# aa2il/pySDR

Measured on AMD Instinct MI355X. Metric: complex IQ MS/s through 4-RX demod chain, higher is better.
Workload: dtype f32; 1 GPU; C3: 8 MS/s synthetic IQ, 4 RX (USB/CW/NFM/AM), 255-tap prototype 3/500, + 64k-FFT RF PSD on every sample; 2048 chunks x 170666 in HBM; parallelism=stream-sharded x1

## Files before the change

include/pysdr_hip.h:

```cpp
#ifndef PYSDR_HIP_H
#define PYSDR_HIP_H

#include <stddef.h>
#include <stdint.h>

#ifdef __cplusplus
extern "C" {
#endif

#define PYSDR_MAX_RX 8

typedef enum {
  PYSDR_OK = 0,
  PYSDR_ERR_ARG = -1,
  PYSDR_ERR_NO_DEVICE = -2,
  PYSDR_ERR_HIP = -3,
  PYSDR_ERR_FFT = -4,
  PYSDR_ERR_STATE = -5,
  PYSDR_ERR_RCCL = -6
} pysdr_status;

typedef enum {
  PYSDR_AM = 0, PYSDR_AM_SYNCH = 1, PYSDR_SSB = 2, PYSDR_USB = 3, PYSDR_LSB = 4,
  PYSDR_CW = 5, PYSDR_IQ = 6, PYSDR_WFM = 7, PYSDR_WFM2 = 8, PYSDR_NFM = 9,
// ... 42 lines not shown
int pysdr_wfm_params(double srate, double fs_out, int* d1, int* up2, int* down2);
int pysdr_set_wfm_taps(pysdr_ctx* ctx, int irx, const double* video, int nv, const double* resamp, int nr);
int pysdr_reset(pysdr_ctx* ctx, int irx, unsigned what);
int pysdr_agc_get(pysdr_ctx* ctx, int irx, pysdr_agc_state* st);
int pysdr_pll_stats(pysdr_ctx* ctx, int irx, int* segments, int* patched);
int pysdr_set_pll_segments(pysdr_ctx* ctx, int max_segments);
int pysdr_pll_join_margin(pysdr_ctx* ctx, int irx, int* max_words, float* max_dw);
int pysdr_pll_linear_starts(pysdr_ctx* ctx, int irx, int* n);
int pysdr_set_squelch(pysdr_ctx* ctx, int irx, float thresh);
int pysdr_squelch_get(pysdr_ctx* ctx, int irx, float* level, int* open);
int pysdr_set_squelch_ratio(pysdr_ctx* ctx, int irx, float min_ratio, const float* lp, const float* hp, int ntaps);
int pysdr_squelch_ratio_get(pysdr_ctx* ctx, int irx, float* sq_lp, float* sq_hp, int* open);
int pysdr_set_agc(pysdr_ctx* ctx, int irx, int enable, float ref);

int pysdr_process(pysdr_ctx* ctx, const float* iq_interleaved, size_t n, pysdr_out* outs);

int pysdr_process_batch(pysdr_ctx* ctx, const void* iq, int nchunks, size_t chunk_len, int on_device);
int pysdr_build_flags_hash(void);
int pysdr_set_overlap(pysdr_ctx* ctx, int enable);
int pysdr_get_overlap(pysdr_ctx* ctx);
int pysdr_last_call_overlapped(pysdr_ctx* ctx);
int pysdr_fetch(pysdr_ctx* ctx, int irx, float* am, float* iq, int cap, int* n_out,
                int* am_is_complex, int* chunk_nout, float* peaks);
int pysdr_sync(pysdr_ctx* ctx);

int pysdr_set_profile(pysdr_ctx* ctx, int enable);
int pysdr_get_elapsed_ms(pysdr_ctx* ctx, int which, int back, float* ms);
int pysdr_set_tile(pysdr_ctx* ctx, int tile_bytes, int threads);
int pysdr_get_tuning(pysdr_ctx* ctx, int32_t out[8]);

#define PYSDR_FORM_VECTOR 0
#define PYSDR_FORM_MFMA 1
#define PYSDR_FORM_SMALL 2
int pysdr_front_end_plan(int nrx, int up, int down, int ntaps, int tile_bytes, int threads, int wgs_per_cu,
                         int yflush_cap, int mfma_enable, int want_peak, int32_t out[12]);
int pysdr_front_end_shapes(int family, int index, int32_t out[4], int* count);

int pysdr_quad_mixer(int device, const float* x, float* y, size_t n, uint32_t phase0,
                     uint32_t fword, uint32_t* phase_out);
uint32_t pysdr_freq_word(double f_hz, double fs_hz, double* f_actual);

int pysdr_fir_real(int device, const float* xx, const float* h, int ntaps, float* y, size_t n);

int  pysdr_spectrum_create(int device, int chunk_size, int nfft, int max_frames,
                           const float* window, pysdr_spectrum** out);
void pysdr_spectrum_destroy(pysdr_spectrum* sp);
int pysdr_spectrum_frame(pysdr_spectrum* sp, const float* x, int is_complex, int db,
                         float* psd_out, int* n_out);
int pysdr_spectrum_batch(pysdr_spectrum* sp, const void* d_iq, int nframes, size_t hop,
                         void* d_out);
int pysdr_spectrum_sync(pysdr_spectrum* sp);
int pysdr_spectrum_get_tuning(pysdr_spectrum* sp, int32_t out[4]);
// ... 59 lines not shown
```

pysdr_amd/_lib.py:

```python
from __future__ import annotations

import ctypes as C
import os

HERE = os.path.dirname(os.path.abspath(__file__))
_variant = os.environ.get("PYSDR_LIB_VARIANT", "") if os.environ.get("PYSDR_TUNING", "0") not in ("", "0") else ""
LIB_PATH = os.path.join(HERE, "libpysdr_hip_diag.so" if os.environ.get("PYSDR_USE_DIAG_LIB") == "1"
                        else (f"libpysdr_hip_{_variant}.so" if _variant else "libpysdr_hip.so"))

MAX_RX = 8


class PysdrError(RuntimeError):
    pass


class Cfg(C.Structure):
    _fields_ = [("srate", C.c_double), ("up", C.c_int32), ("down", C.c_int32),
                ("in_chunk", C.c_int32), ("max_chunks", C.c_int32),
                ("ntaps_dec", C.c_int32), ("ntaps_af", C.c_int32),
                ("device", C.c_int32), ("reserved", C.c_int32)]


class AgcState(C.Structure):
# ... 26 lines not shown
    "pysdr_reset": (_i, [_vp, _i, C.c_uint]),
    "pysdr_agc_get": (_i, [_vp, _i, C.POINTER(AgcState)]),
    "pysdr_pll_stats": (_i, [_vp, _i, _pi, _pi]),
    "pysdr_set_pll_segments": (_i, [_vp, _i]),
    "pysdr_build_flags_hash": (_i, []),
    "pysdr_set_overlap": (_i, [_vp, _i]),
    "pysdr_get_overlap": (_i, [_vp]),
    "pysdr_last_call_overlapped": (_i, [_vp]),
    "pysdr_pll_join_margin": (_i, [_vp, _i, _pi, _pf]),
    "pysdr_pll_linear_starts": (_i, [_vp, _i, _pi]),
    "pysdr_set_agc": (_i, [_vp, _i, _i, _f]),
    "pysdr_set_squelch": (_i, [_vp, _i, _f]),
    "pysdr_squelch_get": (_i, [_vp, _i, _pf, _pi]),
    "pysdr_set_squelch_ratio": (_i, [_vp, _i, _f, _pf, _pf, _i]),
    "pysdr_squelch_ratio_get": (_i, [_vp, _i, _pf, _pf, _pi]),
    "pysdr_process": (_i, [_vp, _pf, _sz, C.POINTER(Out)]),
    "pysdr_process_batch": (_i, [_vp, _vp, _i, _sz, _i]),
    "pysdr_fetch": (_i, [_vp, _i, _pf, _pf, _i, _pi, _pi, _pi, _pf]),
    "pysdr_sync": (_i, [_vp]),
    "pysdr_set_profile": (_i, [_vp, _i]),
    "pysdr_get_elapsed_ms": (_i, [_vp, _i, _i, _pf]),
    "pysdr_set_tile": (_i, [_vp, _i, _i]),
    "pysdr_get_tuning": (_i, [_vp, C.POINTER(C.c_int32)]),
    "pysdr_front_end_plan": (_i, [_i, _i, _i, _i, _i, _i, _i, _i, _i, _i, C.POINTER(C.c_int32)]),
    "pysdr_front_end_shapes": (_i, [_i, _i, C.POINTER(C.c_int32), _pi]),
    "pysdr_quad_mixer": (_i, [_i, _pf, _pf, _sz, _u32, _u32, C.POINTER(_u32)]),
    "pysdr_freq_word": (_u32, [_d, _d, _pd]),
    "pysdr_fir_real": (_i, [_i, _pf, _pf, _i, _pf, _sz]),
    "pysdr_spectrum_create": (_i, [_i, _i, _i, _i, _pf, C.POINTER(_vp)]),
    "pysdr_spectrum_destroy": (None, [_vp]),
    "pysdr_spectrum_frame": (_i, [_vp, _pf, _i, _i, _pf, _pi]),
    "pysdr_spectrum_batch": (_i, [_vp, _vp, _i, _sz, _vp]),
    "pysdr_spectrum_sync": (_i, [_vp]),
    "pysdr_spectrum_get_tuning": (_i, [_vp, C.POINTER(C.c_int32)]),
    "pysdr_spectrum_elapsed_ms": (_i, [_vp, _pf]),
    "pysdr_spectrum_order": (_i, [_vp, _vp, _i]),
    "pysdr_ingest_create": (_i, [_vp, _i, C.POINTER(_vp)]),
    "pysdr_ingest_create_batched": (_i, [_vp, _i, _i, C.POINTER(_vp)]),
    "pysdr_ingest_chunks": (_i, [_vp, _i, _i, _pi, _pi, _pf]),
    "pysdr_ingest_destroy": (None, [_vp]),
    "pysdr_ingest_buffer": (_i, [_vp, _i, C.POINTER(_pf), C.POINTER(C.c_size_t)]),
    "pysdr_ingest_submit": (_i, [_vp, _i, C.c_size_t]),
    "pysdr_ingest_collect": (_i, [_vp, _i, C.POINTER(Out)]),
    "pysdr_waterfall_create": (_i, [_i, _i, _i, C.POINTER(_vp)]),
    "pysdr_waterfall_destroy": (None, [_vp]),
    "pysdr_waterfall_push": (_i, [_vp, _vp, _i, _i]),
# ... 79 lines not shown
```

pysdr_amd/csrc/api.hip:

```cpp
#include <dlfcn.h>
#include <rccl/rccl.h>
#include <rocfft/rocfft.h>

#include <cmath>
#include <algorithm>
#include <cstdarg>
#include <map>

#include "common.h"
#include "host_plan.h"
#include "host_res.h"
#include "mixdec_mfma_geom.h"
#include "mixdec_plan.h"

namespace pysdr {

static thread_local char g_err[2048] = "";

void set_last_error(const char* fmt, ...) {
  va_list ap;
  va_start(ap, fmt);
  vsnprintf(g_err, sizeof(g_err), fmt, ap);
  va_end(ap);
}
// ... 104 lines not shown
  bool use2 = false;
  int par = 0;
  int last_par = 0;
  Event ev_pll[2];
  int n_ingest = 0;
  TailJob tail;
  int hy = 0, mmax = 0;
  size_t cap_samples = 0;
  Decim main;
  Decim wfm_front;
  int d1 = 0, up2 = 0, down2 = 0, m1max = 0;
  int last_wfm = 0;
  DevBuf<float2> d_stage;
  BufPair<unsigned> d_peak2;
  int peak_cur = 0;
  bool peak_clean[2] = {true, true};
#ifdef PYSDR_DIAG
  DevBuf<unsigned long long> d_stamps;
  DevBuf<unsigned long long> d_mm_stamps;
#endif
  DevBuf<unsigned> d_peak_scratch;
  DevBuf<unsigned> d_blkpeak;
  DevBuf<float> d_gain;
  DevBuf<float> d_blknoise;
  DevBuf<float> d_blknoise2;
  DevBuf<float> d_sqtaps;
  int sq_ntaps = 0;
  DevBuf<unsigned> d_blkcnt;
  DevBuf<RxDevState> d_state;
  DevBuf<uint32_t> d_pllseg;
  int last_nout = 0, last_nchunks = 0, last_nrx = 0;
  size_t last_chunk_len = 0;
  unsigned long long last_s0 = 0;
  int last_complex[PYSDR_MAX_RX] = {0};
  Tuning tune;
  int num_cus = 256;
  int pll_kmax = 0;
  int profile = 0;
  static constexpr int kSlots = 64;
  Event ev[kSlots][4];
  Event ev_front;
  hipEvent_t front_marker = nullptr;
  int front_wanted = 0;
  unsigned long long ncalls = 0;
  void* rccl_lib = nullptr;
  ncclComm_t comm = nullptr;
// ... 356 lines not shown
  const double wn = 2.0 * M_PI * kPllBwHz / fs_out;
  s.pll_kp = (float)(2.0 * kPllZeta * wn);
  s.pll_ki = (float)(wn * wn);
  for (int r = 0; r < nrx; ++r) {
    const RxSnap& x = snap.rx[r];
    s.y[r] = x.d_y + c->hy;
    s.ypll[r] = x.d_ypll ? x.d_ypll + c->hy : nullptr;
    s.aftaps[r] = x.d_aftaps;
    s.taps_real[r] = x.taps_real;
    s.a[r] = x.d_a;
    s.am[r] = x.d_am;
    s.det[r] = mode_detector(x.mode);
    s.out_complex[r] = (x.mode == PYSDR_IQ || wfm) ? 1 : 0;
    s.fir_complex[r] = s.out_complex[r];
    s.single_block[r] = wfm ? 1 : 0;
    s.single_spread = 1;
    while (s.single_spread * 2 <= std::min(nchunks, 32)) s.single_spread *= 2;
    s.matrix[r] = (x.mode == PYSDR_WFM2) ? 1 : 0;
    s.bfo_fword[r] = x.bfo_fword;
    s.sq_ratio[r] = (x.sq_ratio > 0.f && c->d_sqtaps) ? 1 : 0;
    s.sq_thresh[r] = s.sq_ratio[r] ? x.sq_ratio : x.sq_thresh;
  }
  s.blkpeak = c->d_blkpeak.get(); s.gain = c->d_gain.get(); s.state = c->d_state.get();
  s.blknoise = c->d_blknoise.get(); s.blkcnt = c->d_blkcnt.get();
  s.blknoise2 = c->d_blknoise2.get(); s.sqtaps = c->d_sqtaps.get(); s.sq_ntaps = c->sq_ntaps;
}

int run_tail(pysdr_ctx* c, TailJob& j) {
  j.valid = false;
  const CallSnap& snap = j.snap;
  const int nrx = snap.nrx;
  if (j.wait_pll) PYSDR_HIP_CHECK(hipStreamWaitEvent(c->stream, c->ev_pll[j.par], 0));
  Stage2Args& s = j.s;
  int rc;
  if (j.wfm) {
    DecimResult res;
    const uint32_t zero = 0u;
    for (int r = 0; r < nrx; ++r) {
      float2* y1 = snap.rx[r].d_y + c->hy;
      rc = decim_run(c, c->rx[r].wfm_audio, snap.rx[r].d_w, (size_t)j.n1, 1, &y1, &zero, &zero, nullptr, 0,
                     c->mmax, &res, c->stream);
      if (rc) return rc;
    }
    fill_stage2(c, snap, true, j.nchunks, j.chunk_len, res, &s);
  }
  const int n_out = s.n_out;
// ... 20 lines not shown
}

int flush_tail(pysdr_ctx* c) {
  if (!c->tail.valid) return PYSDR_OK;
  return run_tail(c, c->tail);
}

int failed_in(const char* entry, int rc) {
  const std::string what = pysdr_last_error();
  set_last_error("%s: %s", entry, what.c_str());
  return rc;
}

int ctx_alloc(pysdr_ctx* c) {
  const pysdr_cfg& cfg = c->cfg;
  const size_t nblk = (size_t)PYSDR_MAX_RX * cfg.max_chunks;
  PYSDR_HIP_CHECK(c->stream.create(hipStreamNonBlocking));
  int rc = decim_init(c->main, cfg.up, cfg.down, cfg.ntaps_dec, PYSDR_MAX_RX, c->stream);
  if (rc) return rc;
  PYSDR_HIP_CHECK(c->d_peak2.alloc_both_zeroed((size_t)cfg.max_chunks, c->stream));
  PYSDR_HIP_CHECK(c->d_peak_scratch.alloc(64));
  PYSDR_HIP_CHECK(c->d_blkpeak.alloc_zeroed(nblk * kBlkStride, c->stream));
  PYSDR_HIP_CHECK(c->d_gain.alloc(nblk));
  PYSDR_HIP_CHECK(c->d_blknoise.alloc_zeroed(nblk * kBlkStride, c->stream));
  PYSDR_HIP_CHECK(c->d_blkcnt.alloc_zeroed(nblk * kBlkStride, c->stream));
  PYSDR_HIP_CHECK(c->d_state.alloc_zeroed(PYSDR_MAX_RX, c->stream));
  PYSDR_HIP_CHECK(c->d_pllseg.alloc((size_t)PYSDR_MAX_RX * kPllSegMax * 5));
  for (int k = 0; k < pysdr_ctx::kSlots; ++k)
    for (int i = 0; i < 4; ++i) PYSDR_HIP_CHECK(c->ev[k][i].create());
  PYSDR_HIP_CHECK(c->ev_front.create(hipEventDisableTiming));
  return PYSDR_OK;
}

int read_rx_state(pysdr_ctx* c, int irx, RxDevState* d) {
  if (!c || irx < 0 || irx >= c->nrx) return PYSDR_ERR_ARG;
  std::lock_guard<std::recursive_mutex> run_lk(c->run_mu);
  int rc = use_device(c->cfg.device);
  if (rc) return rc;
  rc = flush_tail(c);
  if (rc) return rc;
  PYSDR_HIP_CHECK(hipMemcpyAsync(d, c->d_state.get() + irx, sizeof(*d), hipMemcpyDeviceToHost, c->stream));
  PYSDR_HIP_CHECK(hipStreamSynchronize(c->stream));
  return PYSDR_OK;
}

}
// ... 276 lines not shown
#endif

int pysdr_build_flags_hash(void) {
#ifdef PYSDR_EXTRA_FLAGS_HASH
  return (int)(PYSDR_EXTRA_FLAGS_HASH);
#else
  return 0;
#endif
}

int pysdr_get_tuning(pysdr_ctx* c, int32_t out[8]) {
  if (!c || !out) return PYSDR_ERR_ARG;
#ifdef PYSDR_DIAG
  out[0] = 1;
#else
  out[0] = 0;
#endif
  const Tuning& t = c->tune;
  out[1] = t.dbg_flags; out[2] = t.wgs_per_cu; out[3] = t.yflush_cap;
  out[4] = t.tile_bytes; out[5] = t.threads; out[6] = c->num_cus; out[7] = t.mfma_enable;
  return PYSDR_OK;
}

int pysdr_set_profile(pysdr_ctx* c, int enable) {
  if (!c) return PYSDR_ERR_ARG;
  c->profile = enable;
  return PYSDR_OK;
}

int pysdr_set_tile(pysdr_ctx* c, int tile_bytes, int threads) {
  if (!c || (tile_bytes != 0 && (tile_bytes < 4096 || tile_bytes > 150 * 1024)) || threads < 64 || threads > 1024 ||
      (threads & 63))
    return PYSDR_ERR_ARG;
  c->tune.tile_bytes = tile_bytes;
  c->tune.threads = threads;
  return PYSDR_OK;
}

int pysdr_front_end_plan(int nrx, int up, int down, int ntaps, int tile_bytes, int threads, int wgs_per_cu, int yflush_cap,
                         int mfma_enable, int want_peak, int32_t out[12]) {
  if (!out || nrx < 1 || nrx > PYSDR_MAX_RX || up < 1 || down < 1 || ntaps < 1 || wgs_per_cu < 1 || yflush_cap < 0 ||
      (tile_bytes != 0 && (tile_bytes < 4096 || tile_bytes > 150 * 1024)) || threads < 64 || threads > 1024 || (threads & 63))
    return PYSDR_ERR_ARG;
  const int kdec = (ntaps + up - 1) / up;
  MixDecArgs a;
  memset(&a, 0, sizeof(a));
// ... 285 lines not shown
int pysdr_fetch(pysdr_ctx* c, int irx, float* am, float* iq, int cap, int* n_out,
                int* am_is_complex, int* chunk_nout, float* peaks) {
  if (!c || irx < 0 || irx >= c->nrx) return PYSDR_ERR_ARG;
  std::lock_guard<std::recursive_mutex> run_lk(c->run_mu);
  int rc = use_device(c->cfg.device);
  if (rc) return rc;
  rc = flush_tail(c);
  if (rc) return rc;
  const int n = c->last_nout;
  if ((am || iq) && cap < n) { set_last_error("pysdr_fetch: cap %d < n_out %d", cap, n); return PYSDR_ERR_ARG; }
  const int cx = c->last_complex[irx];
  hipStream_t S2 = c->stream;
  const float2* yb = c->rx[irx].d_y.buf(c->last_par);
  if (am && n > 0)
    PYSDR_HIP_CHECK(hipMemcpyAsync(am, c->rx[irx].d_am.get(), (size_t)n * (cx ? 2 : 1) * sizeof(float), hipMemcpyDeviceToHost, S2));
  if (iq && n > 0)
    PYSDR_HIP_CHECK(hipMemcpyAsync(iq, yb + c->hy, (size_t)n * sizeof(float2), hipMemcpyDeviceToHost, S2));
  if (peaks && c->last_nchunks > 0)
    PYSDR_HIP_CHECK(hipMemcpyAsync(peaks, c->d_peak2.buf(c->peak_cur), (size_t)c->last_nchunks * sizeof(float), hipMemcpyDeviceToHost, S2));
  PYSDR_HIP_CHECK(hipStreamSynchronize(S2));
  if (n_out) *n_out = n;
  if (am_is_complex) *am_is_complex = cx;
  if (chunk_nout) last_chunk_counts(c, chunk_nout);
  return PYSDR_OK;
}

int pysdr_process(pysdr_ctx* c, const float* iq, size_t n, pysdr_out* outs) {
  if (!c || !iq || !outs || n < 1) return PYSDR_ERR_ARG;
  std::lock_guard<std::recursive_mutex> run_lk(c->run_mu);
  int rc = pysdr_process_batch(c, iq, 1, n, 0);
  if (rc) return rc;
  rc = flush_tail(c);
  if (rc) return rc;
  for (int r = 0; r < c->last_nrx; ++r) {
    int nout = 0, cx = 0;
    float pk = 0.f;
    rc = pysdr_fetch(c, r, outs[r].am, outs[r].iq, outs[r].cap, &nout, &cx, nullptr, &pk);
    if (rc) return rc;
    outs[r].n_out = nout;
    outs[r].am_is_complex = cx;
    outs[r].peak_in = pk;
  }
  return PYSDR_OK;
}

int pysdr_quad_mixer(int device, const float* x, float* y, size_t n, uint32_t phase0,
// ... 524 lines not shown
```

pysdr_amd/csrc/common.h:

```cpp
#pragma once

#include <hip/hip_runtime.h>

#include <cstdint>
#include <cstdio>
#include <cstring>
#include <mutex>
#include <string>
#include <vector>

#include "../../include/pysdr_hip.h"

#if defined(PYSDR_GLDS_PLAIN)
#define PYSDR_GLDS_POLICY ""
#else
#define PYSDR_GLDS_POLICY " nt"
#endif

namespace pysdr {

void set_last_error(const char* fmt, ...);

#define PYSDR_HIP_CHECK(expr)                                                        \
  do {                                                                               \
// ... 102 lines not shown
#define PYSDR_MFMA_SHAPES(X) \
  X(0, 3, 128, 2, 334, 1, 8, MM_C1_NPROD, MM_C1_NBUF, MM_C1_FLAGS) \
  X(1, 1, 40, MM_C4_S, 255, 1, 8, MM_C4_NPROD, MM_C4_NBUF, MM_C4_FLAGS) \
  X(2, 3, 64, 2, 334, 1, 8, 8, 4, 1 | MM_NTX) \
  X(3, 3, 160, 2, 334, 1, 8, 8, 3, 2 | MM_NTX) \
  X(4, 3, 112, 2, 334, 1, 8, 8, 4, 1 | MM_NTX) \
  X(5, 1, 32, 8, 1001, 1, 8, 4, 3, 0 | MM_NTX) \
  X(6, 1, 40, 6, 1001, 1, 8, 4, 3, 0 | MM_NTX)
inline int mixdec_mfma_shape(int up, int down, int kdec) {
#define PYSDR_MFMA_MATCH(ID, UP, DOWN, S, KT, NB, WK, NP, NBUF, CARRY) \
  if (up == UP && down == DOWN && kdec == KT) return ID;
  PYSDR_MFMA_SHAPES(PYSDR_MFMA_MATCH)
#undef PYSDR_MFMA_MATCH
  return -1;
}
bool mixdec_mfma_plan(int shape, unsigned long long s0, unsigned long long m0, unsigned long long n, MfmaPlan* p);
int launch_mixdec_mfma(int shape, const MixMfmaArgs& a, int grid, hipStream_t st);


#ifndef PYSDR_BLK_STRIDE
#define PYSDR_BLK_STRIDE 16
#endif
constexpr int kBlkStride = PYSDR_BLK_STRIDE;

struct RxDevState {
  float env, gain, maxbuf, err, ref;
  int agc_enable;
  uint32_t pll_phase;
  float pll_w;
  uint32_t wfm_phase;
  float wfm_w;
  float sq_level;
  int sq_open;
  int pll_segments;
  int pll_patched;
  int pll_join_words;
  float pll_join_dw;
  int pll_linear;
  int wfm_slope_ok;
  int wfm_redo;
  double wfm_slope;
  float sq_lp, sq_hp;
};
constexpr int kSqTapsMax = 64;
constexpr float kSqAlpha = 0.001f;
constexpr float kSqLog2Decay = -0.00144341686f;
// ... 23 lines not shown
  float2* ypll[PYSDR_MAX_RX];
  const float2* aftaps[PYSDR_MAX_RX];
  int taps_real[PYSDR_MAX_RX];
  float2* a[PYSDR_MAX_RX];
  float* am[PYSDR_MAX_RX];
  int det[PYSDR_MAX_RX];
  int out_complex[PYSDR_MAX_RX];
  int fir_complex[PYSDR_MAX_RX];
  int fir_rx[PYSDR_MAX_RX];
  uint32_t bfo_fword[PYSDR_MAX_RX];
  int single_block[PYSDR_MAX_RX];
  int single_spread;
  int matrix[PYSDR_MAX_RX];
  float sq_thresh[PYSDR_MAX_RX];
  int sq_ratio[PYSDR_MAX_RX];
  int sq_ntaps;
  const float* sqtaps;
  float* blknoise2;
  float* blknoise;
  unsigned* blkcnt;
  unsigned* blkpeak;
  float* gain;
  RxDevState* state;
  PllPlan pll;
};
int launch_am_phase(const Stage2Args& a, hipStream_t st);
int launch_pll(const Stage2Args& a, hipStream_t st);
int launch_demod_fir(const Stage2Args& a, hipStream_t st);
int launch_apply(const Stage2Args& a, hipStream_t st);

struct EpilogueArgs {
  int nrx, n_out, hy;
  float2* ybase[PYSDR_MAX_RX];
  float2* ydst[PYSDR_MAX_RX];
  float2* ypllbase[PYSDR_MAX_RX];
  float2* yplldst[PYSDR_MAX_RX];
};
int launch_agc_scan(const Stage2Args& a, const EpilogueArgs& e, hipStream_t st);
int launch_hist_roll(const float2* x, const float2* hist_old, float2* hist_new, int hist_len,
                     uint32_t n_total, unsigned* zero, int zero_n, hipStream_t st);

struct WfmArgs {
  int nrx, n1;
  float scale;
  float kp, ki, norm, rad2word;
  uint32_t fword0;
  const float2* y1[PYSDR_MAX_RX];
  float2* y1base[PYSDR_MAX_RX];
// ... 33 lines not shown
```

pysdr_amd/csrc/host_plan.h:

```cpp
#pragma once

#include <algorithm>
#include <cmath>
#include <cstdlib>

#include "common.h"

namespace pysdr {

constexpr double kTwo32 = 4294967296.0;
constexpr double kPllBwHz = 50.0, kPllZeta = 0.7071;
constexpr double kWfmPllBwHz = 30.0;
constexpr int kPllSegMax = 8192;

inline const char* tuning_env(const char* name) {
  const char* on = getenv("PYSDR_TUNING");
  if (!on || atoi(on) <= 0) return nullptr;
  return getenv(name);
}

struct Tuning {
  int tile_bytes = 0, threads = 1024;
  int wgs_per_cu = 1;
  int grid_override = 0;
  int resamp_plain = 0;
  int mfma_enable = 1;
  int dbg_flags = 0, yflush_cap = 0;
  int overlap_env = -1;
  int tail_first = -1;
  bool overlap_prio_set = false;
  int overlap_prio = 0;
  double am_taus = 16.0, am_taus_exact = 5.0;
  int am_coarse_sweeps = 4, am_kmax = 2048, am_tmin = 512;
  int am_seeded = 1, am_wseed = 0;
  int am_direct = 1;
  int am_phase_on_2 = 1;
  double wfm_taus = 20.0, wfm_taus_fast = 13.0, wfm_taus_exact = 4.0;
  int wfm_coarse_sweeps = 3, wfm_kmax = 1536, wfm_tmin = 2048;
  double wfm_taus_hi = 0.0, wfm_taus_mid = 0.0;
  int wfm_tail_cap = 0;
  int wfm_exact_cap = 5;
  int wfm_seeded = 1, wfm_wseed = 0;

  static Tuning from_env() {
    Tuning t;
    { const char* e = tuning_env("PYSDR_MIXDEC_WGS"); if (e && atoi(e) > 0) t.wgs_per_cu = atoi(e); }
    { const char* e = tuning_env("PYSDR_MIXDEC_YFLUSH"); if (e && atoi(e) > 0) t.yflush_cap = atoi(e); }
    { const char* e = tuning_env("PYSDR_AM_PLL");
      if (e && *e) {
        double a = 0, tx = 0; int cs = 0, km = 0, tm = 0;
        const int nf = sscanf(e, "%lf,%lf,%d,%d,%d", &a, &tx, &cs, &km, &tm);
        if (nf >= 1 && a > 0) t.am_taus = a;
        if (nf >= 2 && tx >= 0) t.am_taus_exact = tx;
        if (nf >= 3 && cs >= 0) t.am_coarse_sweeps = std::min(cs, 8);
        if (nf >= 4 && km > 0) t.am_kmax = std::min(km, kPllSegMax);
        if (nf >= 5 && tm >= 64) t.am_tmin = (tm + 63) & ~63;
      } }
    { const char* e = tuning_env("PYSDR_AM_SEED");
      if (e && *e) { int on = 1, ws = 0; const int nf = sscanf(e, "%d,%d", &on, &ws); if (nf >= 1) t.am_seeded = on ? 1 : 0; if (nf >= 2 && ws >= 0) t.am_wseed = ws; } }
    { const char* e = tuning_env("PYSDR_AM_DIRECT"); if (e && *e) t.am_direct = atoi(e) ? 1 : 0; }
    { const char* e = tuning_env("PYSDR_AM_PHASE_STREAM"); if (e && *e) t.am_phase_on_2 = atoi(e) ? 1 : 0; }
    { const char* e = tuning_env("PYSDR_MIXDEC_MFMA"); if (e && *e) t.mfma_enable = atoi(e) ? 1 : 0; }
    { const char* e = tuning_env("PYSDR_WFM_SEED");
      if (e && *e) { int on = 1, ws = 0; const int nf = sscanf(e, "%d,%d", &on, &ws); if (nf >= 1) t.wfm_seeded = on ? 1 : 0; if (nf >= 2 && ws >= 0) t.wfm_wseed = ws; } }
    { const char* e = tuning_env("PYSDR_OVERLAP_ORDER"); if (e && *e) t.tail_first = atoi(e); }
    { const char* e = tuning_env("PYSDR_OVERLAP"); if (e && *e) t.overlap_env = std::max(0, std::min(2, atoi(e))); }
    { const char* e = tuning_env("PYSDR_OVERLAP_PRIO"); if (e && *e) { t.overlap_prio_set = true; t.overlap_prio = atoi(e); } }
    { const char* e = tuning_env("PYSDR_RESAMP_PLAIN"); if (e && *e) t.resamp_plain = atoi(e); }
    { const char* e = tuning_env("PYSDR_MIXDEC_GRID"); if (e && atoi(e) > 0) t.grid_override = atoi(e); }
    { const char* e = tuning_env("PYSDR_WFM_PLL");
      if (e && *e) {
        double a = t.wfm_taus, b = t.wfm_taus_fast, x = t.wfm_taus_exact;
        int sw = t.wfm_coarse_sweeps, km = t.wfm_kmax, tm = t.wfm_tmin, xc = t.wfm_exact_cap;
        double th = t.wfm_taus_hi, tmid = t.wfm_taus_mid;
        int tc = t.wfm_tail_cap;
        const int got = sscanf(e, "%lf,%lf,%lf,%d,%d,%d,%d,%lf,%lf,%d", &a, &b, &x, &sw, &km, &tm, &xc, &th, &tmid, &tc);
        if (got >= 10 && tc >= 0) t.wfm_tail_cap = tc;
        if (got >= 9 && th >= 0 && tmid >= 0) { t.wfm_taus_hi = th; t.wfm_taus_mid = tmid; }
        if (got >= 7 && xc >= 0) t.wfm_exact_cap = xc;
        if (got >= 1 && a > 0) t.wfm_taus = a;
        if (got >= 2 && b >= 0) t.wfm_taus_fast = b;
        if (got >= 3 && x > 0) t.wfm_taus_exact = x;
        if (got >= 4 && sw >= 0) t.wfm_coarse_sweeps = sw;
        if (got >= 5 && km >= 1) t.wfm_kmax = std::min(km, kPllSegMax);
        if (got >= 6 && tm >= 64) t.wfm_tmin = tm;
      } }
#ifdef PYSDR_DIAG
    { const char* e = getenv("PYSDR_DEBUG_FLAGS"); t.dbg_flags = e ? atoi(e) : 0; }
#endif
    return t;
  }
// ... 95 lines not shown
```

pysdr_amd/csrc/stage2.hip:

```cpp
#include "common.h"
#include "hist_roll.h"

namespace pysdr {

namespace {

__device__ __forceinline__ float2 cmul(float2 a, float2 b) {
  return make_float2(a.x * b.x - a.y * b.y, a.x * b.y + a.y * b.x);
}

__device__ __forceinline__ uint32_t block_of(const Stage2Args& a, int r, int i) {
  if (a.single_block[r]) return 0u;
  const uint32_t t = a.t0 + (uint32_t)i * (uint32_t)a.down;
  return (t / (uint32_t)a.up) / a.chunk_len;
}

__device__ __forceinline__ int block_end(const Stage2Args& a, int r, uint32_t b) {
  if (a.single_block[r] || b + 1u >= (uint32_t)a.nchunks) return a.n_out;
  const unsigned long long need = (unsigned long long)(b + 1u) * a.chunk_len * (unsigned)a.up;
  if (need <= a.t0) return 0;
  const unsigned long long i = (need - a.t0 + (unsigned)a.down - 1ull) / (unsigned)a.down;
  return i < (unsigned long long)a.n_out ? (int)i : a.n_out;
}

// ... 670 lines not shown
  __syncthreads();

  float2 acc[kW];
  if (CPLX) {
    fir_run<kFirCplx>(sre, sim, tre, tim, tre_s, tim_s, nblk, H, tid, acc);
  } else {
    const bool real_det = (det == kDetAbs || det == kDetFm || det == kDetPll);
    if (real_det && a.taps_real[r]) fir_run<kFirRealReal>(sre, sim, tre, tim, tre_s, tim_s, nblk, H, tid, acc);
    else fir_run<kFirRePart>(sre, sim, tre, tim, tre_s, tim_s, nblk, H, tid, acc);
  }

  fir_epilogue<CPLX>(a, r, det, i0, H, tid, sre, acc);
}


__device__ __forceinline__ float agc_env_step(float env, float peak) {
  const float dec = __fadd_rn(env, __fmul_rn(0.1f, __fsub_rn(peak, env)));
  return (peak > env) ? peak : dec;
}

__global__ __launch_bounds__(256) void agc_scan_kernel(const Stage2Args a, const EpilogueArgs eh) {
  extern __shared__ __attribute__((aligned(16))) float agc_lds[];
  const int tid = threadIdx.x;
  if ((int)blockIdx.x >= a.nrx) {
    const int job = blockIdx.x - a.nrx;
    const float2* base = (job < eh.nrx) ? eh.ybase[job] : eh.ypllbase[job - eh.nrx];
    float2* dst = (job < eh.nrx) ? eh.ydst[job] : eh.yplldst[job - eh.nrx];
    if (base == nullptr) return;
    float2* sh = reinterpret_cast<float2*>(agc_lds);
    for (int j = tid; j < eh.hy; j += 256) sh[j] = base[eh.n_out + j];
    __syncthreads();
    for (int j = tid; j < eh.hy; j += 256) dst[j] = sh[j];
    return;
  }
  const int r = blockIdx.x;
  const int nch = a.single_block[r] ? (a.nchunks > 0 ? 1 : 0) : a.nchunks;
  const int nacc = a.single_block[r] ? (a.nchunks > 0 ? a.single_spread : 0) : a.nchunks;
  auto px = [](int c) { return c + (c >> 4); };
  const int nlds = px(a.nchunks) + 1;
  float* pk = agc_lds;
  float* ev = agc_lds + nlds;
  float* sS = ev + nlds;
  float* sE = sS + 256;
  for (int c0 = 0; c0 < nacc; c0 += 16 * 256) {
    unsigned v[16];
#pragma unroll
    for (int u = 0; u < 16; ++u) {
      const int c = c0 + u * 256 + tid;
      v[u] = (c < nacc) ? a.blkpeak[((size_t)r * a.nchunks + c) * kBlkStride] : 0u;
    }
#pragma unroll
    for (int u = 0; u < 16; ++u) {
      const int c = c0 + u * 256 + tid;
      if (c < nacc) pk[px(c)] = __uint_as_float(v[u]);
    }
  }
  __syncthreads();
  if (a.single_block[r] && nacc > 1) {
    if (tid == 0) {
      float m = pk[px(0)];
      for (int c = 1; c < nacc; ++c) m = fmaxf(m, pk[px(c)]);
      pk[px(0)] = m;
    }
    __syncthreads();
  }
  const RxDevState st = a.state[r];
  constexpr int kWarm = 176;
  const int T = (nch + 255) / 256 < 16 ? 16 : (nch + 255) / 256;
  const int K = (nch + T - 1) / T;
  if (tid < K) {
    const int s0 = tid * T, s1 = (s0 + T < nch) ? s0 + T : nch;
    int wb = s0 - kWarm;
    float env = 0.f;
    if (tid == 0 || wb <= 0) { wb = 0; env = st.env; }
    int c = wb;
    for (; c + 16 <= s0; c += 16) {
      float v[16];
#pragma unroll
      for (int u = 0; u < 16; ++u) v[u] = pk[px(c + u)];
#pragma unroll
      for (int u = 0; u < 16; ++u) env = agc_env_step(env, v[u]);
    }
    for (; c < s0; ++c) env = agc_env_step(env, pk[px(c)]);
    sS[tid] = env;
    for (c = s0; c + 16 <= s1; c += 16) {
      float v[16];
#pragma unroll
      for (int u = 0; u < 16; ++u) v[u] = pk[px(c + u)];
#pragma unroll
      for (int u = 0; u < 16; ++u) { env = agc_env_step(env, v[u]); ev[px(c + u)] = env; }
    }
    for (; c < s1; ++c) { env = agc_env_step(env, pk[px(c)]); ev[px(c)] = env; }
    sE[tid] = env;
  }
  __syncthreads();
  const bool miss = tid > 0 && tid < K && __float_as_uint(sE[tid - 1]) != __float_as_uint(sS[tid]);
  if (__syncthreads_or(miss) && tid == 0) {
    for (int k = 1; k < K; ++k) {
      if (__float_as_uint(sE[k - 1]) == __float_as_uint(sS[k])) continue;
      float env = sE[k - 1];
      const int s0 = k * T, s1 = (s0 + T < nch) ? s0 + T : nch;
      for (int c = s0; c < s1; ++c) { env = agc_env_step(env, pk[px(c)]); ev[px(c)] = env; }
      sE[k] = env;
      sS[k] = sE[k - 1];
    }
  }
  __syncthreads();
  const float last_peak = nch > 0 ? pk[px(nch - 1)] : st.maxbuf;
  for (int c = tid; c < nch; c += 256) pk[px(c)] = ev[px(c)];
  __syncthreads();
  for (int c = tid; c < nch; c += 256) {
    const float g = st.agc_enable ? fminf(__fdiv_rn(st.ref, fmaxf(pk[px(c)], 1e-12f)), 1.0e4f) : 1.f;
    a.gain[(size_t)r * a.nchunks + c] = g;
    a.blkpeak[((size_t)r * a.nchunks + c) * kBlkStride] = 0u;
  }
  if (a.single_block[r])
    for (int c = 1 + tid; c < nacc; c += 256) a.blkpeak[((size_t)r * a.nchunks + c) * kBlkStride] = 0u;
  const float env_last = nch > 0 ? pk[px(nch - 1)] : 0.f;
  if (a.sq_thresh[r] > 0.f && a.sq_ratio[r]) {
    constexpr int kSqWarm = 32;
    __syncthreads();
    float* wH = ev;
    float* wL = pk;
    float* dk = sE + 256;
    float* lvH = dk + nlds;
    float* lvL = lvH + nlds;
    float* sS2 = lvL + nlds;
    float* sE2 = sS2 + 256;
    for (int c = tid; c < nch; c += 256) {
      const size_t k = ((size_t)r * a.nchunks + c) * kBlkStride;
      const unsigned n = a.blkcnt[k];
// ... 487 lines not shown
                                          hipFuncAttributeMaxDynamicSharedMemorySize, 160 * 1024));
      attr_done |= 1ull << (dev & 63);
    }
  }
  for (int cplx = 0; cplx < 2; ++cplx) {
    Stage2Args b = a;
    int n = 0;
    for (int r = 0; r < a.nrx; ++r)
      if ((a.out_complex[r] ? 1 : 0) == cplx) b.fir_rx[n++] = r;
    if (n == 0) continue;
    dim3 grid((a.n_out + (int)(a.m0_lo & 1u) + kFirOut - 1) / kFirOut, n);
    if (cplx) hipLaunchKernelGGL(demod_fir_kernel<true>, grid, dim3(kFirThreads), lds, st, b);
    else hipLaunchKernelGGL(demod_fir_kernel<false>, grid, dim3(kFirThreads), lds, st, b);
    PYSDR_HIP_CHECK(hipGetLastError());
  }
  return PYSDR_OK;
}

int launch_agc_scan(const Stage2Args& a, const EpilogueArgs& e, hipStream_t st) {
  if (e.hy > 4096) {
    set_last_error("epilogue: history %d too long", e.hy);
    return PYSDR_ERR_ARG;
  }
  const size_t nlds = (size_t)a.nchunks + (a.nchunks >> 4) + 1;
  bool any_ratio = false;
  for (int r = 0; r < a.nrx; ++r) any_ratio |= (a.sq_ratio[r] != 0 && a.sq_thresh[r] > 0.f);
  const size_t lds = std::max(((any_ratio ? 5 : 2) * nlds + (any_ratio ? 1024 : 512)) * sizeof(float), (size_t)e.hy * sizeof(float2));
  if (lds > 48 * 1024) {
    static std::mutex attr_mu;
    static uint64_t attr_done = 0;
    static size_t max_dyn = 0;
    int dev = 0;
    PYSDR_HIP_CHECK(hipGetDevice(&dev));
    std::lock_guard<std::mutex> lk(attr_mu);
    if (max_dyn == 0) {
      hipFuncAttributes fa;
      PYSDR_HIP_CHECK(hipFuncGetAttributes(&fa, reinterpret_cast<const void*>(agc_scan_kernel)));
      max_dyn = (size_t)160 * 1024 - fa.sharedSizeBytes;
    }
    if (lds > max_dyn) { set_last_error("agc: %d blocks per call need %zu bytes of LDS (%zu available)", a.nchunks, lds, max_dyn); return PYSDR_ERR_ARG; }
    if (!((attr_done >> (dev & 63)) & 1ull)) {
      PYSDR_HIP_CHECK(hipFuncSetAttribute(reinterpret_cast<const void*>(agc_scan_kernel),
                                          hipFuncAttributeMaxDynamicSharedMemorySize, (int)max_dyn));
      attr_done |= 1ull << (dev & 63);
    }
  }
  hipLaunchKernelGGL(agc_scan_kernel, dim3(a.nrx + 2 * e.nrx), dim3(256), lds, st, a, e);
  PYSDR_HIP_CHECK(hipGetLastError());
  return PYSDR_OK;
}

int launch_apply(const Stage2Args& a, hipStream_t st) {
  if (a.n_out <= 0) return PYSDR_OK;
  dim3 grid((a.n_out + 1023) / 1024, a.nrx);
  hipLaunchKernelGGL(apply_kernel, grid, dim3(256), 0, st, a);
  PYSDR_HIP_CHECK(hipGetLastError());
  return PYSDR_OK;
}

int launch_hist_roll(const float2* x, const float2* hist_old, float2* hist_new, int hist_len,
                     uint32_t n_total, unsigned* zero, int zero_n, hipStream_t st) {
  hipLaunchKernelGGL(hist_roll_kernel, dim3(1), dim3(256), 0, st, x, hist_old, hist_new, hist_len, n_total, zero, zero_n);
  PYSDR_HIP_CHECK(hipGetLastError());
  return PYSDR_OK;
}

int launch_wfm_disc(const WfmArgs& a, hipStream_t st) {
  if (a.n1 > 0) {
    hipLaunchKernelGGL(wfm_disc_kernel, dim3((a.n1 + kSeedTile - 1) / kSeedTile, a.nrx), dim3(256), 0, st, a);
    PYSDR_HIP_CHECK(hipGetLastError());
// ... 41 lines not shown
```

Baseline: 118,300 MS/s.

## Split AGC envelope scan across several workgroups per receiver with last-block join

```diff
diff --git a/include/pysdr_hip.h b/include/pysdr_hip.h
--- a/include/pysdr_hip.h
+++ b/include/pysdr_hip.h
@@ -88,12 +88,14 @@
 int pysdr_last_call_overlapped(pysdr_ctx* ctx);
 int pysdr_fetch(pysdr_ctx* ctx, int irx, float* am, float* iq, int cap, int* n_out,
                 int* am_is_complex, int* chunk_nout, float* peaks);
+int pysdr_fetch_gains(pysdr_ctx* ctx, int irx, float* gains, int cap, int* nblocks);
 int pysdr_sync(pysdr_ctx* ctx);
 
 int pysdr_set_profile(pysdr_ctx* ctx, int enable);
 int pysdr_get_elapsed_ms(pysdr_ctx* ctx, int which, int back, float* ms);
 int pysdr_set_tile(pysdr_ctx* ctx, int tile_bytes, int threads);
 int pysdr_get_tuning(pysdr_ctx* ctx, int32_t out[8]);
+int pysdr_get_agc_scan(pysdr_ctx* ctx, int32_t out[4]);
 
 #define PYSDR_FORM_VECTOR 0
 #define PYSDR_FORM_MFMA 1
diff --git a/pysdr_amd/_lib.py b/pysdr_amd/_lib.py
--- a/pysdr_amd/_lib.py
+++ b/pysdr_amd/_lib.py
@@ -72,6 +72,8 @@
     "pysdr_get_elapsed_ms": (_i, [_vp, _i, _i, _pf]),
     "pysdr_set_tile": (_i, [_vp, _i, _i]),
     "pysdr_get_tuning": (_i, [_vp, C.POINTER(C.c_int32)]),
+    "pysdr_get_agc_scan": (_i, [_vp, C.POINTER(C.c_int32)]),
+    "pysdr_fetch_gains": (_i, [_vp, _i, _pf, _i, _pi]),
     "pysdr_front_end_plan": (_i, [_i, _i, _i, _i, _i, _i, _i, _i, _i, _i, C.POINTER(C.c_int32)]),
     "pysdr_front_end_shapes": (_i, [_i, _i, C.POINTER(C.c_int32), _pi]),
     "pysdr_quad_mixer": (_i, [_i, _pf, _pf, _sz, _u32, _u32, C.POINTER(_u32)]),
diff --git a/pysdr_amd/csrc/api.hip b/pysdr_amd/csrc/api.hip
--- a/pysdr_amd/csrc/api.hip
+++ b/pysdr_amd/csrc/api.hip
@@ -150,6 +150,9 @@
   DevBuf<unsigned> d_peak_scratch;
   DevBuf<unsigned> d_blkpeak;
   DevBuf<float> d_gain;
+  DevBuf<float> d_agcenv;
+  DevBuf<float> d_agcseg;
+  DevBuf<unsigned> d_agcjoin;
   DevBuf<float> d_blknoise;
   DevBuf<float> d_blknoise2;
   DevBuf<float> d_sqtaps;
@@ -552,6 +555,9 @@
     s.sq_thresh[r] = s.sq_ratio[r] ? x.sq_ratio : x.sq_thresh;
   }
   s.blkpeak = c->d_blkpeak.get(); s.gain = c->d_gain.get(); s.state = c->d_state.get();
+  s.agc_ranges = agc_scan_ranges(nchunks, c->tune.agc_ranges);
+  s.agc_env = c->d_agcenv.get(); s.agc_seg = c->d_agcseg.get();
+  s.agc_join = c->d_agcjoin.get(); s.agc_diag = c->d_agcjoin.get() + PYSDR_MAX_RX * kAgcJoinPitch;
   s.blknoise = c->d_blknoise.get(); s.blkcnt = c->d_blkcnt.get();
   s.blknoise2 = c->d_blknoise2.get(); s.sqtaps = c->d_sqtaps.get(); s.sq_ntaps = c->sq_ntaps;
 }
@@ -618,6 +624,9 @@
   PYSDR_HIP_CHECK(c->d_peak_scratch.alloc(64));
   PYSDR_HIP_CHECK(c->d_blkpeak.alloc_zeroed(nblk * kBlkStride, c->stream));
   PYSDR_HIP_CHECK(c->d_gain.alloc(nblk));
+  PYSDR_HIP_CHECK(c->d_agcenv.alloc(nblk));
+  PYSDR_HIP_CHECK(c->d_agcseg.alloc((size_t)PYSDR_MAX_RX * 2 * kAgcSegMax));
+  PYSDR_HIP_CHECK(c->d_agcjoin.alloc_zeroed((size_t)PYSDR_MAX_RX * kAgcJoinPitch + kAgcDiagWords, c->stream));
   PYSDR_HIP_CHECK(c->d_blknoise.alloc_zeroed(nblk * kBlkStride, c->stream));
   PYSDR_HIP_CHECK(c->d_blkcnt.alloc_zeroed(nblk * kBlkStride, c->stream));
   PYSDR_HIP_CHECK(c->d_state.alloc_zeroed(PYSDR_MAX_RX, c->stream));
@@ -940,6 +949,20 @@
   return PYSDR_OK;
 }
 
+int pysdr_get_agc_scan(pysdr_ctx* c, int32_t out[4]) {
+  if (!c || !out) return PYSDR_ERR_ARG;
+  std::lock_guard<std::recursive_mutex> run_lk(c->run_mu);
+  int rc = use_device(c->cfg.device);
+  if (rc) return rc;
+  rc = flush_tail(c);
+  if (rc) return rc;
+  unsigned diag[kAgcDiagWords];
+  PYSDR_HIP_CHECK(hipMemcpyAsync(diag, c->d_agcjoin.get() + PYSDR_MAX_RX * kAgcJoinPitch, sizeof(diag), hipMemcpyDeviceToHost, c->stream));
+  PYSDR_HIP_CHECK(hipStreamSynchronize(c->stream));
+  out[0] = c->tune.agc_ranges; out[1] = (int32_t)diag[0]; out[2] = (int32_t)diag[1]; out[3] = 0;
+  return PYSDR_OK;
+}
+
 int pysdr_set_profile(pysdr_ctx* c, int enable) {
   if (!c) return PYSDR_ERR_ARG;
   c->profile = enable;
@@ -1271,6 +1294,22 @@
   if (n_out) *n_out = n;
   if (am_is_complex) *am_is_complex = cx;
   if (chunk_nout) last_chunk_counts(c, chunk_nout);
+  return PYSDR_OK;
+}
+
+int pysdr_fetch_gains(pysdr_ctx* c, int irx, float* gains, int cap, int* nblocks) {
+  if (!c || irx < 0 || irx >= c->nrx) return PYSDR_ERR_ARG;
+  std::lock_guard<std::recursive_mutex> run_lk(c->run_mu);
+  int rc = use_device(c->cfg.device);
+  if (rc) return rc;
+  rc = flush_tail(c);
+  if (rc) return rc;
+  const int n = c->last_wfm ? (c->last_nchunks > 0 ? 1 : 0) : c->last_nchunks;
+  if (gains && cap < n) { set_last_error("pysdr_fetch_gains: cap %d < %d blocks", cap, n); return PYSDR_ERR_ARG; }
+  if (gains && n > 0)
+    PYSDR_HIP_CHECK(hipMemcpyAsync(gains, c->d_gain.get() + (size_t)irx * c->last_nchunks, (size_t)n * sizeof(float), hipMemcpyDeviceToHost, c->stream));
+  PYSDR_HIP_CHECK(hipStreamSynchronize(c->stream));
+  if (nblocks) *nblocks = n;
   return PYSDR_OK;
 }
 
diff --git a/pysdr_amd/csrc/common.h b/pysdr_amd/csrc/common.h
--- a/pysdr_amd/csrc/common.h
+++ b/pysdr_amd/csrc/common.h
@@ -148,6 +148,7 @@
 #define PYSDR_BLK_STRIDE 16
 #endif
 constexpr int kBlkStride = PYSDR_BLK_STRIDE;
+static_assert(kBlkStride >= 2 && kBlkStride % 2 == 0, "PYSDR_BLK_STRIDE: an even number of words, at least 2");
 
 struct RxDevState {
   float env, gain, maxbuf, err, ref;
@@ -217,8 +218,21 @@
   unsigned* blkpeak;
   float* gain;
   RxDevState* state;
+  int agc_ranges;
+  float* agc_env;
+  float* agc_seg;
+  unsigned* agc_join;
+  unsigned* agc_diag;
   PllPlan pll;
 };
+constexpr int kAgcSegMax = 256;
+constexpr int kAgcJoinPitch = 32;
+constexpr int kAgcDiagWords = 4;
+constexpr int kAgcRangesMax = 8;
+inline int agc_scan_ranges(int nchunks, int forced) {
+  const int j = forced > 0 ? forced : nchunks / 256;
+  return j < 1 ? 1 : (j > kAgcRangesMax ? kAgcRangesMax : j);
+}
 int launch_am_phase(const Stage2Args& a, hipStream_t st);
 int launch_pll(const Stage2Args& a, hipStream_t st);
 int launch_demod_fir(const Stage2Args& a, hipStream_t st);
diff --git a/pysdr_amd/csrc/host_plan.h b/pysdr_amd/csrc/host_plan.h
--- a/pysdr_amd/csrc/host_plan.h
+++ b/pysdr_amd/csrc/host_plan.h
@@ -24,6 +24,7 @@
   int wgs_per_cu = 1;
   int grid_override = 0;
   int resamp_plain = 0;
+  int agc_ranges = 0;
   int mfma_enable = 1;
   int dbg_flags = 0, yflush_cap = 0;
   int overlap_env = -1;
@@ -67,6 +68,7 @@
     { const char* e = tuning_env("PYSDR_OVERLAP"); if (e && *e) t.overlap_env = std::max(0, std::min(2, atoi(e))); }
     { const char* e = tuning_env("PYSDR_OVERLAP_PRIO"); if (e && *e) { t.overlap_prio_set = true; t.overlap_prio = atoi(e); } }
     { const char* e = tuning_env("PYSDR_RESAMP_PLAIN"); if (e && *e) t.resamp_plain = atoi(e); }
+    { const char* e = tuning_env("PYSDR_AGC_RANGES"); if (e && atoi(e) > 0) t.agc_ranges = atoi(e); }
     { const char* e = tuning_env("PYSDR_MIXDEC_GRID"); if (e && atoi(e) > 0) t.grid_override = atoi(e); }
     { const char* e = tuning_env("PYSDR_WFM_PLL");
       if (e && *e) {
diff --git a/pysdr_amd/csrc/stage2.hip b/pysdr_amd/csrc/stage2.hip
--- a/pysdr_amd/csrc/stage2.hip
+++ b/pysdr_amd/csrc/stage2.hip
@@ -716,8 +716,9 @@
 __global__ __launch_bounds__(256) void agc_scan_kernel(const Stage2Args a, const EpilogueArgs eh) {
   extern __shared__ __attribute__((aligned(16))) float agc_lds[];
   const int tid = threadIdx.x;
-  if ((int)blockIdx.x >= a.nrx) {
-    const int job = blockIdx.x - a.nrx;
+  const int J = a.agc_ranges;
+  if ((int)blockIdx.x >= a.nrx * J) {
+    const int job = blockIdx.x - a.nrx * J;
     const float2* base = (job < eh.nrx) ? eh.ybase[job] : eh.ypllbase[job - eh.nrx];
     float2* dst = (job < eh.nrx) ? eh.ydst[job] : eh.yplldst[job - eh.nrx];
     if (base == nullptr) return;
@@ -727,7 +728,7 @@
     for (int j = tid; j < eh.hy; j += 256) dst[j] = sh[j];
     return;
   }
-  const int r = blockIdx.x;
+  const int r = blockIdx.x / J, j = blockIdx.x - r * J;
   const int nch = a.single_block[r] ? (a.nchunks > 0 ? 1 : 0) : a.nchunks;
   const int nacc = a.single_block[r] ? (a.nchunks > 0 ? a.single_spread : 0) : a.nchunks;
   auto px = [](int c) { return c + (c >> 4); };
@@ -736,19 +737,32 @@
   float* ev = agc_lds + nlds;
   float* sS = ev + nlds;
   float* sE = sS + 256;
-  for (int c0 = 0; c0 < nacc; c0 += 16 * 256) {
-    unsigned v[16];
-#pragma unroll
-    for (int u = 0; u < 16; ++u) {
-      const int c = c0 + u * 256 + tid;
-      v[u] = (c < nacc) ? a.blkpeak[((size_t)r * a.nchunks + c) * kBlkStride] : 0u;
-    }
-#pragma unroll
-    for (int u = 0; u < 16; ++u) {
-      const int c = c0 + u * 256 + tid;
-      if (c < nacc) pk[px(c)] = __uint_as_float(v[u]);
-    }
-  }
+  auto load_peaks = [&](int lo, int hi) {
+    for (int c0 = lo; c0 < hi; c0 += 16 * 256) {
+      unsigned v[16];
+#pragma unroll
+      for (int u = 0; u < 16; ++u) {
+        const int c = c0 + u * 256 + tid;
+        v[u] = (c < hi) ? a.blkpeak[((size_t)r * a.nchunks + c) * kBlkStride] : 0u;
+      }
+#pragma unroll
+      for (int u = 0; u < 16; ++u) {
+        const int c = c0 + u * 256 + tid;
+        if (c < hi) pk[px(c)] = __uint_as_float(v[u]);
+      }
+    }
+  };
+  constexpr int kWarm = 176;
+  const int T = (nch + 255) / 256 < 16 ? 16 : (nch + 255) / 256;
+  const int K = (nch + T - 1) / T;
+  const int jr = (a.single_block[r] || K < 2) ? 1 : (J < K ? J : K);
+  const int spr = (K + jr - 1) / jr;
+  const int nranges = spr > 0 ? (K + spr - 1) / spr : 1;
+  if (j >= nranges) return;
+  const int k0 = j * spr, k1 = (k0 + spr < K) ? k0 + spr : K;
+  const int lo = (nranges > 1 && k0 * T > kWarm) ? k0 * T - kWarm : 0;
+  const int hi = (nranges > 1) ? ((k1 * T < nch) ? k1 * T : nch) : nacc;
+  load_peaks(lo, hi);
   __syncthreads();
   if (a.single_block[r] && nacc > 1) {
     if (tid == 0) {
@@ -759,14 +773,12 @@
     __syncthreads();
   }
   const RxDevState st = a.state[r];
-  constexpr int kWarm = 176;
-  const int T = (nch + 255) / 256 < 16 ? 16 : (nch + 255) / 256;
-  const int K = (nch + T - 1) / T;
-  if (tid < K) {
-    const int s0 = tid * T, s1 = (s0 + T < nch) ? s0 + T : nch;
+  if (tid < k1 - k0) {
+    const int k = k0 + tid;
+    const int s0 = k * T, s1 = (s0 + T < nch) ? s0 + T : nch;
     int wb = s0 - kWarm;
     float env = 0.f;
-    if (tid == 0 || wb <= 0) { wb = 0; env = st.env; }
+    if (k == 0 || wb <= 0) { wb = 0; env = st.env; }
     int c = wb;
     for (; c + 16 <= s0; c += 16) {
       float v[16];
@@ -776,7 +788,7 @@
       for (int u = 0; u < 16; ++u) env = agc_env_step(env, v[u]);
     }
     for (; c < s0; ++c) env = agc_env_step(env, pk[px(c)]);
-    sS[tid] = env;
+    sS[k] = env;
     for (c = s0; c + 16 <= s1; c += 16) {
       float v[16];
 #pragma unroll
@@ -785,22 +797,70 @@
       for (int u = 0; u < 16; ++u) { env = agc_env_step(env, v[u]); ev[px(c + u)] = env; }
     }
     for (; c < s1; ++c) { env = agc_env_step(env, pk[px(c)]); ev[px(c)] = env; }
-    sE[tid] = env;
+    sE[k] = env;
   }
   __syncthreads();
+  if (nranges > 1) {
+    __shared__ int is_last;
+    float* genv = a.agc_env + (size_t)r * a.nchunks;
+    float* gS = a.agc_seg + (size_t)r * 2 * kAgcSegMax, *gE = gS + kAgcSegMax;
+    unsigned* join = a.agc_join + (size_t)r * kAgcJoinPitch;
+    for (int c = k0 * T + tid; c < hi; c += 256) __hip_atomic_store(genv + c, ev[px(c)], __ATOMIC_RELAXED, __HIP_MEMORY_SCOPE_AGENT);
+    if (tid < k1 - k0) {
+      __hip_atomic_store(gS + k0 + tid, sS[k0 + tid], __ATOMIC_RELAXED, __HIP_MEMORY_SCOPE_AGENT);
+      __hip_atomic_store(gE + k0 + tid, sE[k0 + tid], __ATOMIC_RELAXED, __HIP_MEMORY_SCOPE_AGENT);
+    }
+    asm volatile("s_waitcnt vmcnt(0)" ::: "memory");
+    __syncthreads();
+    if (tid == 0) is_last = (__hip_atomic_fetch_add(join, 1u, __ATOMIC_RELAXED, __HIP_MEMORY_SCOPE_AGENT) == (unsigned)(nranges - 1)) ? 1 : 0;
+    __syncthreads();
+    if (!is_last) return;
+    if (tid == 0) {
+      __hip_atomic_store(join, 0u, __ATOMIC_RELAXED, __HIP_MEMORY_SCOPE_AGENT);
+      atomicAdd(a.agc_diag + 1, 1u);
+    }
+    const bool other = tid < K && (tid < k0 || tid >= k1);
+    const float oS = other ? __hip_atomic_load(gS + tid, __ATOMIC_RELAXED, __HIP_MEMORY_SCOPE_AGENT) : 0.f;
+    const float oE = other ? __hip_atomic_load(gE + tid, __ATOMIC_RELAXED, __HIP_MEMORY_SCOPE_AGENT) : 0.f;
+    for (int c0 = 0; c0 < nch; c0 += 16 * 256) {
+      float v[16];
+#pragma unroll
+      for (int u = 0; u < 16; ++u) {
+        const int c = c0 + u * 256 + tid;
+        v[u] = (c < nch && (c < k0 * T || c >= hi)) ? __hip_atomic_load(genv + c, __ATOMIC_RELAXED, __HIP_MEMORY_SCOPE_AGENT) : 0.f;
+      }
+#pragma unroll
+      for (int u = 0; u < 16; ++u) {
+        const int c = c0 + u * 256 + tid;
+        if (c < nch && (c < k0 * T || c >= hi)) ev[px(c)] = v[u];
+      }
+    }
+    if (other) { sS[tid] = oS; sE[tid] = oE; }
+    __syncthreads();
+  }
   const bool miss = tid > 0 && tid < K && __float_as_uint(sE[tid - 1]) != __float_as_uint(sS[tid]);
-  if (__syncthreads_or(miss) && tid == 0) {
-    for (int k = 1; k < K; ++k) {
-      if (__float_as_uint(sE[k - 1]) == __float_as_uint(sS[k])) continue;
-      float env = sE[k - 1];
-      const int s0 = k * T, s1 = (s0 + T < nch) ? s0 + T : nch;
-      for (int c = s0; c < s1; ++c) { env = agc_env_step(env, pk[px(c)]); ev[px(c)] = env; }
-      sE[k] = env;
-      sS[k] = sE[k - 1];
+  if (__syncthreads_or(miss)) {
+    if (nranges > 1) {
+      load_peaks(0, nch);
+      __syncthreads();
+    }
+    if (tid == 0) {
+      unsigned redone = 0u;
+      for (int k = 1; k < K; ++k) {
+        if (__float_as_uint(sE[k - 1]) == __float_as_uint(sS[k])) continue;
+        float env = sE[k - 1];
+        const int s0 = k * T, s1 = (s0 + T < nch) ? s0 + T : nch;
+        for (int c = s0; c < s1; ++c) { env = agc_env_step(env, pk[px(c)]); ev[px(c)] = env; }
+        sE[k] = env;
+        sS[k] = sE[k - 1];
+        ++redone;
+      }
+      atomicAdd(a.agc_diag, redone);
     }
   }
   __syncthreads();
-  const float last_peak = nch > 0 ? pk[px(nch - 1)] : st.maxbuf;
+  const float last_peak = nch <= 0 ? st.maxbuf
+                        : nranges > 1 ? __uint_as_float(a.blkpeak[((size_t)r * a.nchunks + nch - 1) * kBlkStride]) : pk[px(nch - 1)];
   for (int c = tid; c < nch; c += 256) pk[px(c)] = ev[px(c)];
   __syncthreads();
   for (int c = tid; c < nch; c += 256) {
@@ -1334,10 +1394,15 @@
     set_last_error("epilogue: history %d too long", e.hy);
     return PYSDR_ERR_ARG;
   }
+  if (a.agc_ranges < 1 || a.agc_ranges > kAgcRangesMax) {
+    set_last_error("agc: %d workgroups per RX", a.agc_ranges);
+    return PYSDR_ERR_ARG;
+  }
   const size_t nlds = (size_t)a.nchunks + (a.nchunks >> 4) + 1;
   bool any_ratio = false;
   for (int r = 0; r < a.nrx; ++r) any_ratio |= (a.sq_ratio[r] != 0 && a.sq_thresh[r] > 0.f);
-  const size_t lds = std::max(((any_ratio ? 5 : 2) * nlds + (any_ratio ? 1024 : 512)) * sizeof(float), (size_t)e.hy * sizeof(float2));
+  size_t lds = std::max(((any_ratio ? 5 : 2) * nlds + (any_ratio ? 1024 : 512)) * sizeof(float), (size_t)e.hy * sizeof(float2));
+  if (a.agc_ranges > 1) lds = std::max(lds, (size_t)84 * 1024);
   if (lds > 48 * 1024) {
     static std::mutex attr_mu;
     static uint64_t attr_done = 0;
@@ -1357,7 +1422,7 @@
       attr_done |= 1ull << (dev & 63);
     }
   }
-  hipLaunchKernelGGL(agc_scan_kernel, dim3(a.nrx + 2 * e.nrx), dim3(256), lds, st, a, e);
+  hipLaunchKernelGGL(agc_scan_kernel, dim3(a.nrx * a.agc_ranges + 2 * e.nrx), dim3(256), lds, st, a, e);
   PYSDR_HIP_CHECK(hipGetLastError());
   return PYSDR_OK;
 }
```

Result: no change. 117,300 MS/s (-0.8%).
